# 10258392511/InverseProblemWithDiffusionModel

Hardware: AMD Instinct MI355X
Metric: ALD reconstructions/sec (128x128 complex, R=40, 4-coil) (higher is better)
Workload: dtype f32 (convolutions: operands as two fp16 pieces = 22 significand bits + 2 signs, three fp16 MFMAs per product, fp32 accumulate; every image scaled into fp16's range by an exact power of two from its producer's per-image maxima: any fp32 input, DESIGN.md 4.2); 1 GPU; ACDC-style 128x128 complex SENSE R=40 4-coil ALD reconstruction, NCSNv2Deepest ngf=128 (94.1M params, seeded random init), sigma 348->0.01 x 2311 levels x 3 steps, L2Penalty, denoise; 14 posterior samples = 14 on rank 0 + 13 per further rank (the 105-sample / 8-GPU partition of BASELINE config 3); samples_total=14, samples_this_rank=14, parallelism=sample-sharded x1, hip_graph=True, state_finite=True

## Files before the change

include/ipdm.h:

```cpp
#ifndef IPDM_H
#define IPDM_H

#include <stddef.h>
#include <stdint.h>

#ifdef __cplusplus
extern "C" {
#endif

#define IPDM_OK 0
#define IPDM_EINVAL (-1)
#define IPDM_EUNSUPPORTED (-2)

#define IPDM_ACT_NONE 0
#define IPDM_ACT_ELU 1
#define IPDM_ACT_RELU 2
#define IPDM_ACT_LRELU02 3
#define IPDM_ACT_SWISH 4
#define IPDM_ACT_COPY 5

#define IPDM_AMAX_WAYS 8
#define IPDM_AMAX_SLOT 128

#define IPDM_ABI_VERSION 4
// ... 215 lines not shown
                           int64_t n_samples, int64_t sample_elems, void* stream);

int ipdm_philox_normal_f32(float* out, uint64_t seed, int64_t sample_offset, int64_t step_id, int plane,
                           int64_t n_samples, int64_t sample_elems, void* stream);

int ipdm_philox_block_host(uint64_t seed, int64_t sample, int64_t step_id, int plane, uint32_t quad, uint32_t* out4);


int ipdm_instnorm_plus_coef_f32(const float* x, const float* alpha, const float* gamma, const float* beta,
                                float* coef, int B, int C, int HW,
                                float* amax_bound ,
                                void* stream);
int ipdm_cond_instnorm_plus_coef_f32(const float* x, const float* embed, const int64_t* labels, int num_classes, int bias,
                                     float* coef, int B, int C, int HW, float* amax_bound, void* stream);
int ipdm_affine_act_f32(const float* x, const float* coef, float* y, int B, int C, int HW, int act, void* stream);
int ipdm_act_f32(const float* x, float* y, int64_t n, int act, void* stream);
int ipdm_scale_shift_f32(const float* x, float* y, int64_t n, float a, float b, void* stream);
int ipdm_add_f32(const float* x, const float* y, float* out, int64_t n, void* stream);
int ipdm_div_sigma_f32(const float* x, const float* sigmas, const int64_t* labels, float* out,
                       int B, int64_t sample_elems, void* stream);
int ipdm_conv3x3_thin_supported(int Cin, int Cout, int H, int W);
int ipdm_conv3x3_thin_f32(const float* x, const float* w, const float* bias,
                          const float* coef ,
                          float* out, int B, int Cin, int Cout, int H, int W, void* stream);
int ipdm_conv3x3_thin_stats_partials(int Cin, int Cout, int H, int W);
int ipdm_conv3x3_thin_stats_f32(const float* x, const float* w, const float* bias, const float* coef, float* out, float* part,
                                int B, int Cin, int Cout, int H, int W, void* stream);
int ipdm_conv3x3_fewout_fin_supported(int Cin, int Cout, int H, int W);
int ipdm_conv3x3_fewout_fin_f32(const float* x, const float* w, const float* bias, const float* coef, int act, float* out,
                                int B, int Cin, int Cout, int H, int W, void* stream);
// ... 89 lines not shown
int ipdm_conv2d_wino_bx3_stats_partials(int Cin, int Cout, int H, int W, int dilation, int pool2);
int ipdm_conv2d_wino_bx3_stats_f32(const float* x, const void* U, const float* bias, const float* residual, float* out,
                                   float* out_act, int act_out, int B, int Cin, int Cout, int H, int W, int dilation,
                                   int pool2, float* stats, const ipdm_conv_ext_t* ext, void* stream);
int ipdm_absmax_f32(const float* x, float* amax , int n_images,
                    int64_t per_image, void* stream);
int64_t ipdm_conv_hx2_weight_bytes(int Cout, int Cin, int k);
int ipdm_conv_hx2_pack_weight(const float* w , void* packed, int Cout,
                              int Cin, int k, void* stream);
int ipdm_conv2d_hx2_f32(const float* x, const void* packed, const float* bias, const float* coef, int act,
                        const float* residual, float* out, float* out_act, int act_out,
                        int B, int Cin, int Cout, int H, int W, int k, int dilation, const ipdm_conv_ext_t* ext, void* stream);
int ipdm_conv3d_hx2_f32(const float* x, const void* packed, const float* bias, const float* coef, int act,
                        const float* residual, float* out, float* out_act, int act_out,
                        int B, int Cin, int Cout, int D, int H, int W, int k, int dilation, const ipdm_conv_ext_t* ext, void* stream);
int ipdm_conv_hx2_splitk_f32(const float* x, const void* packed, const float* bias, const float* coef, int act,
                             const float* residual, float* out, float* out_act, int act_out,
                             int B, int Cin, int Cout, int D, int H, int W, int k, int dilation, int volume, int ksplit,
                             float* work, const ipdm_conv_ext_t* ext, void* stream);
int64_t ipdm_conv_wino_hx2_weight_bytes(int Cout, int Cin);
int ipdm_conv_wino_hx2_pack_weight(const float* w , void* U, int Cout, int Cin, void* stream);
int ipdm_conv2d_wino_hx2_f32(const float* x, const void* U, const float* bias, const float* residual, float* out,
                             float* out_act, int act_out, int B, int Cin, int Cout, int H, int W, int dilation,
                             int pool2, const ipdm_conv_ext_t* ext, void* stream);
#define IPDM_WINO_FORM_OTHER 0
#define IPDM_WINO_FORM_CO32 1
#define IPDM_WINO_FORM_HALF 2
#define IPDM_WINO_FORM_POLY 3
int ipdm_conv2d_wino_hx2_form(int Cin, int Cout, int H, int W, int dilation);
int64_t ipdm_conv_wino1d_weight_bytes(int Cout, int Cin);
// ... 69 lines not shown
```

inverseproblemwithdiffusionmodel_amd/_lib.py:

```python
import ctypes
import os

import torch
from ctypes import c_char_p, c_double, c_float, c_int, c_int64, c_uint64, c_void_p


class ConvExt(ctypes.Structure):
    _fields_ = [("in_amax", c_void_p), ("bias_bstride", c_int), ("out_scale", c_float), ("res_second", c_int),
                ("out_amax", c_void_p), ("act_amax", c_void_p)]


_HERE = os.path.dirname(os.path.abspath(__file__))
LIB_PATH = os.environ.get("IPDM_LIB") or os.path.join(_HERE, "libipdm.so")

P = c_void_p

SIGNATURES = {
    "ipdm_abi_version": [],
    "ipdm_build_arch": [],
    "ipdm_upfirdn2d_f32": [P, P, P] + [c_int] * 14 + [P],
    "ipdm_fused_bias_act_f32": [P, P, P, P, c_int64, c_int, c_int, c_int, c_int, c_float, c_float, P],
    "ipdm_upfirdn2d_f16": [P, P, P] + [c_int] * 14 + [P],
    "ipdm_upfirdn2d_f64": [P, P, P] + [c_int] * 14 + [P],
    "ipdm_fused_bias_act_f16": [P, P, P, P, c_int64, c_int, c_int, c_int, c_int, c_float, c_float, P],
# ... 62 lines not shown
    "ipdm_pc_langevin_coef_f32": [P, P, P, P, c_double, c_double, c_uint64, c_int64, c_int64, P, c_float, c_float, P, P,
                                  c_int, c_int64, P],
    "ipdm_pc_sense_step_f32": [P, P, P, P, P, P, c_float, c_float, c_uint64, c_int64, c_int64, P, c_int,
                               P, P, c_int, c_int, P, c_int, c_float, P, c_int, c_int, c_int, c_int, P],
    "ipdm_pc_sense_cg_step_f32": [P, P, P, P, P, P, c_float, c_float, c_uint64, c_int64, c_int64, P, c_int,
                                  P, P, c_int, c_int, P, c_int, c_float, P, P, c_int, c_float, P,
                                  c_int, c_int, c_int, c_int, P],
    "ipdm_pc_singlecoil_step_f32": [P, P, P, P, P, P, c_float, c_float, c_uint64, c_int64, c_int64, P, c_int,
                                    P, P, c_int, c_float, c_int, P, c_int, c_int, c_int, P],
    "ipdm_langevin_step_f32": [P, P, P, c_float, c_float, c_uint64, c_int64, c_int64, P, c_int64, c_int64, P],
    "ipdm_philox_normal_f32": [P, c_uint64, c_int64, c_int64, c_int, c_int64, c_int64, P],
    "ipdm_philox_block_host": [c_uint64, c_int64, c_int64, c_int, ctypes.c_uint32, P],
    "ipdm_instnorm_plus_coef_f32": [P, P, P, P, P, c_int, c_int, c_int, P, P],
    "ipdm_cond_instnorm_plus_coef_f32": [P, P, P, c_int, c_int, P, c_int, c_int, c_int, P, P],
    "ipdm_affine_act_f32": [P, P, P, c_int, c_int, c_int, c_int, P],
    "ipdm_act_f32": [P, P, c_int64, c_int, P],
    "ipdm_scale_shift_f32": [P, P, c_int64, c_float, c_float, P],
    "ipdm_add_f32": [P, P, P, c_int64, P],
    "ipdm_div_sigma_f32": [P, P, P, P, c_int, c_int64, P],
    "ipdm_maxpool5_f32": [P, P, c_int, c_int, c_int, P],
    "ipdm_affine_avgpool5_f32": [P, P, P, c_int, c_int, c_int, P],
    "ipdm_meanpool2_f32": [P, P, c_int, c_int, c_int, P],
    "ipdm_bilinear_f32": [P, P, c_int, c_int, c_int, c_int, c_int, c_int, c_int, c_int, P, P],
    "ipdm_conv3x3_thin_supported": [c_int, c_int, c_int, c_int],
    "ipdm_conv3x3_thin_f32": [P, P, P, P, P, c_int, c_int, c_int, c_int, c_int, P],
    "ipdm_conv3x3_thin_stats_partials": [c_int, c_int, c_int, c_int],
    "ipdm_conv3x3_thin_stats_f32": [P, P, P, P, P, P, c_int, c_int, c_int, c_int, c_int, P],
    "ipdm_conv3x3_fewout_fin_supported": [c_int, c_int, c_int, c_int],
    "ipdm_conv3x3_fewout_fin_f32": [P, P, P, P, c_int, P, c_int, c_int, c_int, c_int, c_int, P],
    "ipdm_trilinear_f32": [P, P, c_int, c_int, c_int, c_int, c_int, c_int, c_int, c_int, c_int, c_int, P, P],
# ... 24 lines not shown
    "ipdm_conv_bx3_splitk_f32": [P, P, P, P, c_int, P, P, P, c_int] + [c_int] * 10 + [P, P, P],
    "ipdm_adam_ascent_f32": [P, P, P, P, c_int64, c_float, c_float, c_float, c_float, c_int, P],
    "ipdm_conv_wino_bx3_weight_bytes": [c_int, c_int],
    "ipdm_conv_wino_bx3_pack_weight": [P, P, c_int, c_int, P],
    "ipdm_conv2d_wino_bx3_supported": [c_int, c_int, c_int, c_int, c_int],
    "ipdm_conv2d_wino_bx3_f32": [P, P, P, P, P, P, c_int, c_int, c_int, c_int, c_int, c_int, c_int, c_int, P, P],
    "ipdm_conv2d_wino_bx3_stats_partials": [c_int, c_int, c_int, c_int, c_int, c_int],
    "ipdm_conv2d_wino_bx3_splitk": [c_int, c_int, c_int, c_int, c_int],
    "ipdm_conv2d_wino_bx3_splitk_f32": [P, P, P, P, P, P, c_int, c_int, c_int, c_int, c_int, c_int, c_int, c_int, P, P, P],
    "ipdm_conv2d_wino_bx3_stats_f32": [P, P, P, P, P, P, c_int, c_int, c_int, c_int, c_int, c_int, c_int, c_int, P, P, P],
    "ipdm_conv_hx2_weight_bytes": [c_int, c_int, c_int],
    "ipdm_conv_hx2_pack_weight": [P, P, c_int, c_int, c_int, P],
    "ipdm_absmax_f32": [P, P, c_int, c_int64, P],
    "ipdm_conv2d_hx2_f32": [P, P, P, P, c_int, P, P, P, c_int] + [c_int] * 7 + [P, P],
    "ipdm_conv3d_hx2_f32": [P, P, P, P, c_int, P, P, P, c_int] + [c_int] * 8 + [P, P],
    "ipdm_conv_hx2_splitk_f32": [P, P, P, P, c_int, P, P, P, c_int] + [c_int] * 10 + [P, P, P],
    "ipdm_conv_wino_hx2_weight_bytes": [c_int, c_int],
    "ipdm_conv_wino1d_weight_bytes": [c_int, c_int],
    "ipdm_conv_wino1d_pack_weight": [P, P, c_int, c_int, P],
    "ipdm_conv2d_wino1d_supported": [c_int, c_int, c_int, c_int],
    "ipdm_conv_wino1d_weight_bytes3d": [c_int, c_int],
    "ipdm_conv_wino1d_pack_weight3d": [P, P, c_int, c_int, P],
    "ipdm_conv3d_wino1d_supported": [c_int, c_int, c_int, c_int, c_int],
    "ipdm_conv3d_wino1d_f32": [P, P, P, P, P, P, c_int, c_int, c_int, c_int, c_int, c_int, c_int, P, P],
    "ipdm_conv2d_wino1d_f32": [P, P, P, P, c_int, P, P, P, c_int, c_int, c_int, c_int, c_int, c_int, c_int, P, P],
    "ipdm_conv2d_wino1d_stats_partials": [c_int, c_int, c_int, c_int],
    "ipdm_conv2d_wino1d_stats_f32": [P, P, P, P, c_int, P, P, P, c_int, c_int, c_int, c_int, c_int, c_int, c_int, P, P, P],
    "ipdm_conv_wino_hx2_pack_weight": [P, P, c_int, c_int, P],
    "ipdm_conv2d_wino_hx2_f32": [P, P, P, P, P, P, c_int, c_int, c_int, c_int, c_int, c_int, c_int, c_int, P, P],
    "ipdm_conv2d_wino_hx2_form": [c_int] * 5,
# ... 74 lines not shown
```

inverseproblemwithdiffusionmodel_amd/csrc/conv_bx3.hip:

```cpp
#include "conv_kernel.h"

namespace ipdm_conv {

constexpr int BX3_KG = 8;

template <int NCT, int NPT, int WCO, int WPX, int PW, int DMAX, int KS, bool HX = false, int ZT = 1>
struct BxCfg {
  static constexpr int NPC = HX ? 2 : 3;
  static constexpr int TAPS = KS * KS;
  static constexpr int CO_T = 32 * NCT * WCO;
  static constexpr int ROWS_PER_TILE = 32 / PW;
  static constexpr int PH = NPT * WPX * ROWS_PER_TILE;
  static constexpr int HALO = KS == 3 ? DMAX : 0;
  static constexpr int PHP = PH + 2 * HALO;
  static constexpr int PWP = PW + 2 * HALO;
  static constexpr int PITCH = PW == 32 ? PWP : (PWP + 15) / 16 * 16;
  static constexpr int PLANE_S = PHP * PITCH;
  static constexpr int PLANE = ZT * PLANE_S;
  static constexpr int STAGE = 2 * NPC * PLANE;
  static constexpr int ITEMS = (2 * ZT * PHP * PWP + 255) / 256;
  static constexpr int NPT_T = NPT * ZT;
  static constexpr size_t LDS_BYTES = 2 * (size_t)STAGE * 16;
};

// ... 718 lines not shown
```

inverseproblemwithdiffusionmodel_amd/csrc/conv_kernel.h:

```cpp
#pragma once
#include "launch.h"
#include <cstddef>
#include <cstdlib>
#include <type_traits>
#include <utility>

namespace ipdm_conv {

typedef float f32x16 __attribute__((ext_vector_type(16)));
typedef __bf16 bf16x8 __attribute__((ext_vector_type(8)));

__device__ __forceinline__ void split3(const float (&v)[8], bf16x8& h, bf16x8& m, bf16x8& l) {
#pragma unroll
  for (int i = 0; i < 8; ++i) {
    const __bf16 hi = (__bf16)v[i];
    const float r1 = v[i] - (float)hi;
    const __bf16 mi = (__bf16)r1;
    const float r2 = r1 - (float)mi;
    h[i] = hi;
    m[i] = mi;
    l[i] = (__bf16)r2;
  }
}

// ... 47 lines not shown
  (f(std::integral_constant<int, Is>{}), ...);
}
template <int N, typename F>
__device__ __forceinline__ void static_for(F&& f) {
  static_for_impl(f, std::make_integer_sequence<int, N>{});
}

__device__ __forceinline__ float half_wave_sum(float v) {
  v += __builtin_bit_cast(float, __builtin_amdgcn_update_dpp(0, __builtin_bit_cast(int, v), 0xB1, 0xf, 0xf, false));
  v += __builtin_bit_cast(float, __builtin_amdgcn_update_dpp(0, __builtin_bit_cast(int, v), 0x4E, 0xf, 0xf, false));
  v += __builtin_bit_cast(float, __builtin_amdgcn_update_dpp(0, __builtin_bit_cast(int, v), 0x141, 0xf, 0xf, false));
  v += __builtin_bit_cast(float, __builtin_amdgcn_update_dpp(0, __builtin_bit_cast(int, v), 0x140, 0xf, 0xf, false));
  return v + __shfl_xor(v, 16, 64);
}


struct ConvArgs {
  const float* x = nullptr;
  const float* wt = nullptr;
  const float* bias = nullptr;
  const float* coef = nullptr;
  const float* residual = nullptr;
  float* out = nullptr;
  float* out_act = nullptr;
  int act_out = IPDM_ACT_NONE;
  int B = 0, Cin = 0, Cout = 0, H = 0, W = 0, dil = 1, act = IPDM_ACT_NONE;
  int D = 1, kd = 1;
  int tiles_x = 0, tiles_y = 0, co_tiles = 0;
  unsigned long long* dbg = nullptr;
  int pool2 = 0;
// ... 392 lines not shown
```

inverseproblemwithdiffusionmodel_amd/csrc/norm_act.hip:

```cpp
#include "ipdm_common.h"

namespace {

template <bool REG>
__global__ __launch_bounds__(256) void plane_stats_kernel(const float* __restrict__ x, float* __restrict__ coef,
                                                          int HW) {
  __shared__ double red[4];
  const float* p = x + (size_t)blockIdx.x * HW;
  const int tid = threadIdx.x, lane = tid & 63, wave = tid >> 6;
  const bool vec = REG || ((HW % 4 == 0) && ((reinterpret_cast<uintptr_t>(p) & 15) == 0));
  float4 keep[16];
  float s = 0.f;
  if constexpr (REG) {
    const int n4 = HW / 4;
#pragma unroll
    for (int k = 0; k < 16; ++k) {
      const int i = tid + k * 256;
      keep[k] = i < n4 ? reinterpret_cast<const float4*>(p)[i] : make_float4(0.f, 0.f, 0.f, 0.f);
    }
#pragma unroll
    for (int k = 0; k < 16; ++k)
      if (tid + k * 256 < n4) s += (keep[k].x + keep[k].y) + (keep[k].z + keep[k].w);
  } else if (vec) {
    for (int i = tid; i < HW / 4; i += 256) {
// ... 174 lines not shown
  const size_t plane = blockIdx.y;
  const float mu = coef[plane * 3], sc = coef[plane * 3 + 1], sh = coef[plane * 3 + 2];
  const float* p = x + plane * HW;
  float* o = y + plane * HW;
  if ((HW & 3) == 0 && ((reinterpret_cast<uintptr_t>(p) | reinterpret_cast<uintptr_t>(o)) & 15) == 0) {
    for (int i = blockIdx.x * 256 + threadIdx.x; i < HW / 4; i += gridDim.x * 256) {
      float4 v = reinterpret_cast<const float4*>(p)[i];
      v.x = ipdm_act((v.x - mu) * sc + sh, act);
      v.y = ipdm_act((v.y - mu) * sc + sh, act);
      v.z = ipdm_act((v.z - mu) * sc + sh, act);
      v.w = ipdm_act((v.w - mu) * sc + sh, act);
      reinterpret_cast<float4*>(o)[i] = v;
    }
  } else {
    for (int i = blockIdx.x * 256 + threadIdx.x; i < HW; i += gridDim.x * 256) o[i] = ipdm_act((p[i] - mu) * sc + sh, act);
  }
}

__global__ __launch_bounds__(256) void affine_act_cat_kernel(const float* x1, int C1, const float* x2, int C2,
                                                             const float* __restrict__ coef, float* y, int HW, int act) {
  const size_t plane = blockIdx.y;
  const int Ct = C1 + C2;
  const size_t b = plane / Ct;
  const int c = (int)(plane % Ct);
  const float mu = coef[plane * 3], sc = coef[plane * 3 + 1], sh = coef[plane * 3 + 2];
  const float* p = c < C1 ? x1 + (b * C1 + c) * HW : x2 + (b * C2 + (c - C1)) * HW;
  float* o = y + plane * HW;
  if ((HW & 3) == 0 && ((reinterpret_cast<uintptr_t>(p) | reinterpret_cast<uintptr_t>(o)) & 15) == 0) {
    for (int i = blockIdx.x * 256 + threadIdx.x; i < HW / 4; i += gridDim.x * 256) {
      float4 v = reinterpret_cast<const float4*>(p)[i];
// ... 389 lines not shown
  if (B == 0) return IPDM_OK;
  IPDM_REQUIRE(x && coef && y);
  IPDM_REQUIRE((int64_t)B * C <= 65535 * 32);
  int gx = (HW / 4 + 255) / 256;
  if (gx < 1) gx = 1;
  if (gx > 64) gx = 64;
  int64_t planes = (int64_t)B * C;
  for (int64_t p0 = 0; p0 < planes; p0 += 65535) {
    int np = (int)((planes - p0) < 65535 ? (planes - p0) : 65535);
    hipLaunchKernelGGL(affine_act_kernel, dim3(gx, np), dim3(256), 0, ipdm_stream(stream), x + p0 * HW, coef + p0 * 3,
                       y + p0 * HW, HW, act);
  }
  return ipdm_launch_status();
}

extern "C" int ipdm_affine_act_cat_f32(const float* x1, int C1, const float* x2, int C2, const float* coef, float* y, int B,
                                       int HW, int act, void* stream) {
  IPDM_REQUIRE(B >= 0 && C1 > 0 && C2 > 0 && HW > 0);
  if (B == 0) return IPDM_OK;
  IPDM_REQUIRE(x1 && x2 && coef && y && y != x1 && y != x2);
  const int64_t planes = (int64_t)B * (C1 + C2);
  if (planes > 65535) return IPDM_EUNSUPPORTED;
  int gx = (HW / 4 + 255) / 256;
  gx = gx < 1 ? 1 : (gx > 64 ? 64 : gx);
  hipLaunchKernelGGL(affine_act_cat_kernel, dim3(gx, (unsigned)planes), dim3(256), 0, ipdm_stream(stream), x1, C1, x2, C2, coef,
                     y, HW, act);
  return ipdm_launch_status();
}

extern "C" int ipdm_act_f32(const float* x, float* y, int64_t n, int act, void* stream) {
// ... 174 lines not shown
```

inverseproblemwithdiffusionmodel_amd/ncsn/models/layers.py:

```python
import os
from functools import partial

import torch
import torch.nn as nn

from ... import ops, _lib
from .normalization import InstanceNorm2dPlus, ConditionalInstanceNorm2dPlus, get_normalization


class _Act:

    def __init__(self, name):
        self.name = name
        self.code = ops.ACT_CODES[name]

    def __call__(self, x):
        return ops.act(x, self.code)


USE_WINOGRAD = os.environ.get("IPDM_WINOGRAD", "1") != "0"
FUSE_POOL = os.environ.get("IPDM_FUSE_POOL", "1") != "0"


def get_act(config):
# ... 131 lines not shown
def _maxpool(x):
    if x.dim() == 3:
        return ops.maxpool1d5(x)
    return ops.maxpool3d5(x) if x.dim() == 5 else ops.maxpool5(x)


class ConvMeanPool(nn.Module):
    def __init__(self, input_dim, output_dim, kernel_size=3, biases=True, adjust_padding=False, spec_norm=False, ndim=2):
        super().__init__()
        if adjust_padding or spec_norm:
            raise NotImplementedError("adjust_padding / spec_norm are unused by every shipped config")
        if ndim == 3:
            raise NotImplementedError("the 8-way 3-D ConvMeanPool is unused by NCSN3DShallow (all its stages are dilated)")
        self.conv = Conv2d(input_dim, output_dim, kernel_size, bias=biases, ndim=ndim)

    def forward(self, inputs, feeds_conv=True):
        if self.conv.ndim == 1:
            if self.conv.kernel_size == 1:
                return self.conv(ops.meanpool1d2(inputs), feeds_conv=feeds_conv)
            return ops.meanpool1d2(self.conv(inputs, feeds_conv=feeds_conv))
        if self.conv.kernel_size == 1:
            return self.conv(ops.meanpool2(inputs), feeds_conv=feeds_conv)
        return ops.meanpool2(self.conv(inputs, feeds_conv=feeds_conv))

    def fused(self, inputs, residual=None, act_out=ops.ACT_NONE, feeds_conv=True, coef=None, act=ops.ACT_NONE):
        c = self.conv
        route = c.route(inputs, site="pool", coef=coef, act=act, act_out=act_out)
        bias, dyn = None if c.bias is None else c.bias.data, ops.dynamic_range()
        if route is None:
            return None
        if route == ops.ROUTE_SEQ:
            return ops.conv1d(inputs, c.packed_conv1d(), bias, residual, c.dilation,
                              act_out=act_out, in_amax=ops.in_amax_for(inputs) if dyn else None, want_amax=dyn and feeds_conv,
                              pool2=True)
        try:
            if coef is not None:
                return ops.conv2d_wino_bx3(inputs, c.packed_wino1d(), bias, residual,
# ... 156 lines not shown
                self.normalize2 = normalization(output_dim)
                self.conv2 = dilated_conv3x3_(output_dim, output_dim, dilation=dilation, spec_norm=spec_norm)
            else:
                conv_shortcut = partial(conv1x1_, spec_norm=spec_norm)
                self.conv1 = conv3x3_(input_dim, output_dim, spec_norm=spec_norm)
                self.normalize2 = normalization(output_dim)
                self.conv2 = conv3x3_(output_dim, output_dim, spec_norm=spec_norm)
        else:
            raise Exception('invalid resample value')
        if output_dim != input_dim or resample is not None:
            self.shortcut = conv_shortcut(input_dim, output_dim)
        self.normalize1 = normalization(input_dim)

    def forward(self, x, want_act=False):
        code = _act_code(self.non_linearity)
        h = self._norm_act_conv(self.normalize1, self.conv1, x, code, want_stats=True, feeds_conv=False)
        a2 = None
        if self.output_dim == self.input_dim and self.resample is None:
            shortcut = x
        else:
            shortcut = self.shortcut(x, feeds_conv=False)
        if isinstance(self.conv2, ConvMeanPool):
            plain_norm = isinstance(self.normalize2, InstanceNorm2dPlus) and self.conv2.conv.ndim == 2
            coef2 = self.normalize2.coef(h) if plain_norm else None
            fin = plain_norm and code == ops.ACT_ELU and self.conv2.conv.fuses_input(h, coef2)
            a2 = h if fin else (ops.affine_act(h, coef2, code) if plain_norm else self.normalize2(h, code))
            fused = self.conv2.fused(a2, residual=shortcut, act_out=code if want_act else ops.ACT_NONE, feeds_conv=want_act,
                                     coef=coef2 if fin else None, act=code if fin else ops.ACT_NONE)
            if fused is not None:
                return fused
            if fin:
                a2 = ops.affine_act(h, coef2, code)
            out = ops.add(shortcut, self.conv2(a2))
            return (out, ops.act(out, code)) if want_act else out
        if want_act:
            return self._norm_act_conv(self.normalize2, self.conv2, h, code, residual=shortcut, act_out=code, want_stats=True)
        return self._norm_act_conv(self.normalize2, self.conv2, h, code, residual=shortcut, want_stats=True, feeds_conv=False)

    @staticmethod
    def _norm_act_conv(norm, conv, x, code, **kw):
        if code == ops.ACT_ELU and isinstance(conv, Conv2d) and conv.ndim == 2 and isinstance(norm, InstanceNorm2dPlus):
            coef = norm.coef(x)
            if conv.fuses_input(x, coef):
                return conv(x, coef=coef, act=code, **kw)
            return conv(ops.affine_act(x, coef, code), **kw)
        return conv(norm(x, code), **kw)



def _cond_norm_act_conv(coef, conv, x, code, **kw):
    if code == ops.ACT_ELU and isinstance(conv, Conv2d) and conv.fuses_input(x, coef):
        return conv(x, coef=coef, act=code, **kw)
    return conv(ops.affine_act(x, coef, code), **kw)


class ConditionalResidualBlock(nn.Module):
    def __init__(self, input_dim, output_dim, num_classes, resample=None, act=None,
                 normalization=ConditionalInstanceNorm2dPlus, adjust_padding=False, dilation=None, spec_norm=False):
        super().__init__()
        self.non_linearity = act
        self.input_dim = input_dim
# ... 166 lines not shown
```

inverseproblemwithdiffusionmodel_amd/ops.py:

```python
import ctypes
import os

import torch

from . import _lib
from ._lib import call, P

ACT_NONE, ACT_ELU, ACT_RELU, ACT_LRELU02, ACT_SWISH = 0, 1, 2, 3, 4
ACT_COPY = 5
CONV_TRACE = None

ACT_CODES = {"none": ACT_NONE, None: ACT_NONE, "elu": ACT_ELU, "relu": ACT_RELU, "lrelu": ACT_LRELU02,
             "swish": ACT_SWISH}


def _gpu(t, dtype=None, name="tensor"):
    if not isinstance(t, torch.Tensor) or not t.is_cuda:
        raise RuntimeError(f"ipdm: {name} must be a GPU tensor (the HIP path has no CPU fallback); got "
                           f"{getattr(t, 'device', type(t))}")
    if dtype is not None and t.dtype != dtype:
        raise TypeError(f"ipdm: {name} must be {dtype}, got {t.dtype}")
    return t if t.is_contiguous() else t.contiguous()


# ... 1240 lines not shown
    part = getattr(x, "_ipdm_partials", None)
    if part is not None:
        del x._ipdm_partials
        part, tag = part
        if tag != (x._version, x.data_ptr()):
            part = None
    if part is not None and USE_STATS_EPILOGUE and tuple(part.shape[:2]) == (B, C):
        call("ipdm_cond_instnorm_plus_coef_partials_f32", _ptr(part), int(part.shape[2]), _ptr(embed), _ptr(labels), nc,
             int(bool(bias)), _ptr(coef), B, C, hw, _ptr(bound), _stream())
        return coef
    call("ipdm_cond_instnorm_plus_coef_f32", _ptr(x), _ptr(embed), _ptr(labels), nc, int(bool(bias)), _ptr(coef), B, C, hw,
         _ptr(bound), _stream())
    return coef


def affine_act(x, coef, act=ACT_NONE, out=None):
    x = _gpu(x, torch.float32, "x")
    B, C = x.shape[:2]
    out = torch.empty_like(x) if out is None else out
    call("ipdm_affine_act_f32", _ptr(x), _ptr(coef), _ptr(out), B, C, x.numel() // max(B * C, 1), act, _stream())
    _written(out)
    return tag_amax(out, getattr(coef, "_ipdm_amax_bound", None))


def act(x, code, out=None):
    x = _gpu(x, torch.float32, "x")
    out = torch.empty_like(x) if out is None else out
    call("ipdm_act_f32", _ptr(x), _ptr(out), x.numel(), code, _stream())
    am = amax_of(x)
    _written(out)
    return tag_amax(out, am)


def scale_shift(x, a, b, out=None):
    x = _gpu(x, torch.float32, "x")
    out = torch.empty_like(x) if out is None else out
    call("ipdm_scale_shift_f32", _ptr(x), _ptr(out), x.numel(), float(a), float(b), _stream())
# ... 554 lines not shown
        D = 1
    ksplit = _lib.lib.ipdm_conv_bx3_splitk(B, D, Cin, wq.Cout, H, W, k, dilation) if B else 1
    if ksplit > 1:
        work = torch.empty((ksplit,) + shape, dtype=torch.float32, device=x.device)
        call(f"ipdm_conv_{wq.fmt}_splitk_f32", _ptr(x), _ptr(wq.blob), _ptr(bias), _ptr(coef), act, _ptr(residual), _ptr(out),
             _ptr(out_act), act_out, B, Cin, wq.Cout, D, H, W, k, dilation, int(vol), ksplit, _ptr(work), ext, _stream())
    elif vol:
        call(f"ipdm_conv3d_{wq.fmt}_f32", _ptr(x), _ptr(wq.blob), _ptr(bias), _ptr(coef), act, _ptr(residual), _ptr(out),
             _ptr(out_act), act_out, B, Cin, wq.Cout, D, H, W, k, dilation, ext, _stream())
    else:
        call(f"ipdm_conv2d_{wq.fmt}_f32", _ptr(x), _ptr(wq.blob), _ptr(bias), _ptr(coef), act, _ptr(residual), _ptr(out),
             _ptr(out_act), act_out, B, Cin, wq.Cout, H, W, k, dilation, ext, _stream())
    _written(out)
    return _conv_done(e0, out, out_act, slot_o, slot_a, B=B * D, Cin=Cin, Cout=wq.Cout, H=H, W=W, k=k, dil=dilation, bx3=True,
                      fmt=wq.fmt, res=residual is not None, taps3d=wq.kk if vol else None)


def conv_wino_bx3_weight(w, fmt="bx3"):
    if fmt not in SPLIT_IMPLS:
        raise ValueError(f"conv_wino_bx3_weight: fmt {fmt!r}")
    w = _gpu(w, torch.float32, "weight")
    Cout, Cin = w.shape[:2]
    nbytes = getattr(_lib.lib, f"ipdm_conv_wino_{fmt}_weight_bytes")(Cout, Cin)
    blob = torch.empty(nbytes, dtype=torch.uint8, device=w.device)
    call(f"ipdm_conv_wino_{fmt}_pack_weight", _ptr(w), _ptr(blob), Cout, Cin, _stream())
    return PackedBx3(blob, Cout, Cin, 16, fmt)


def conv_wino_hx2_weight(w):
    return conv_wino_bx3_weight(w, fmt="hx2")
# ... 331 lines not shown
```

Measured before the change: 0.1257 reconstructions/s.

## Fuse shortcut meanpool into norm-act pass and add streaming 1x1 conv kernel

On downsampling residual blocks, the norm+ELU affine pass now also emits the 2x2 mean-pooled raw input, so the separate meanpool over the block input is dropped. The pooled tensor then goes to a new streaming 1x1 fp16x2 MFMA conv kernel that stages input channels through LDS, instead of the generic conv path. Both are on by default behind environment flags. The aim is to cut one full read of the activation and launch overhead on the shortcut branch, at the cost of a new kernel with its own tiling and precision path.

New measurement: 0.1268 reconstructions/s (median of 6 runs). No clear change (+0.8%).

```diff
diff --git a/include/ipdm.h b/include/ipdm.h
--- a/include/ipdm.h
+++ b/include/ipdm.h
@@ -253,6 +253,8 @@
 int ipdm_cond_instnorm_plus_coef_f32(const float* x, const float* embed, const int64_t* labels, int num_classes, int bias,
                                      float* coef, int B, int C, int HW, float* amax_bound, void* stream);
 int ipdm_affine_act_f32(const float* x, const float* coef, float* y, int B, int C, int HW, int act, void* stream);
+int ipdm_affine_act_pool2_f32(const float* x, const float* coef, float* y, float* pooled, int B, int C, int H, int W, int act,
+                              void* stream);
 int ipdm_act_f32(const float* x, float* y, int64_t n, int act, void* stream);
 int ipdm_scale_shift_f32(const float* x, float* y, int64_t n, float a, float b, void* stream);
 int ipdm_add_f32(const float* x, const float* y, float* out, int64_t n, void* stream);
@@ -372,6 +374,8 @@
 int ipdm_conv3d_hx2_f32(const float* x, const void* packed, const float* bias, const float* coef, int act,
                         const float* residual, float* out, float* out_act, int act_out,
                         int B, int Cin, int Cout, int D, int H, int W, int k, int dilation, const ipdm_conv_ext_t* ext, void* stream);
+int ipdm_conv1x1_stream_hx2_f32(const float* x, const void* packed, const float* bias, float* out, int B, int Cin, int Cout,
+                                int H, int W, const ipdm_conv_ext_t* ext, void* stream);
 int ipdm_conv_hx2_splitk_f32(const float* x, const void* packed, const float* bias, const float* coef, int act,
                              const float* residual, float* out, float* out_act, int act_out,
                              int B, int Cin, int Cout, int D, int H, int W, int k, int dilation, int volume, int ksplit,
diff --git a/inverseproblemwithdiffusionmodel_amd/_lib.py b/inverseproblemwithdiffusionmodel_amd/_lib.py
--- a/inverseproblemwithdiffusionmodel_amd/_lib.py
+++ b/inverseproblemwithdiffusionmodel_amd/_lib.py
@@ -100,6 +100,7 @@
     "ipdm_instnorm_plus_coef_f32": [P, P, P, P, P, c_int, c_int, c_int, P, P],
     "ipdm_cond_instnorm_plus_coef_f32": [P, P, P, c_int, c_int, P, c_int, c_int, c_int, P, P],
     "ipdm_affine_act_f32": [P, P, P, c_int, c_int, c_int, c_int, P],
+    "ipdm_affine_act_pool2_f32": [P, P, P, P, c_int, c_int, c_int, c_int, c_int, P],
     "ipdm_act_f32": [P, P, c_int64, c_int, P],
     "ipdm_scale_shift_f32": [P, P, c_int64, c_float, c_float, P],
     "ipdm_add_f32": [P, P, P, c_int64, P],
@@ -154,6 +155,7 @@
     "ipdm_absmax_f32": [P, P, c_int, c_int64, P],
     "ipdm_conv2d_hx2_f32": [P, P, P, P, c_int, P, P, P, c_int] + [c_int] * 7 + [P, P],
     "ipdm_conv3d_hx2_f32": [P, P, P, P, c_int, P, P, P, c_int] + [c_int] * 8 + [P, P],
+    "ipdm_conv1x1_stream_hx2_f32": [P, P, P, P, c_int, c_int, c_int, c_int, c_int, P, P],
     "ipdm_conv_hx2_splitk_f32": [P, P, P, P, c_int, P, P, P, c_int] + [c_int] * 10 + [P, P, P],
     "ipdm_conv_wino_hx2_weight_bytes": [c_int, c_int],
     "ipdm_conv_wino1d_weight_bytes": [c_int, c_int],
diff --git a/inverseproblemwithdiffusionmodel_amd/csrc/conv1x1_stream.hip b/inverseproblemwithdiffusionmodel_amd/csrc/conv1x1_stream.hip
--- /dev/null
+++ b/inverseproblemwithdiffusionmodel_amd/csrc/conv1x1_stream.hip
@@ -0,0 +1,212 @@
+#include "conv_kernel.h"
+
+namespace ipdm_conv {
+
+struct Conv1x1Args {
+  const float* x;
+  const uint4* wq;
+  const float* bias;
+  const float* in_amax;
+  float* out;
+  float out_scale;
+  int B, Cin, Cout, HW;
+  int n_pt, n_cg;
+};
+
+constexpr int S1_KB = 8;
+constexpr int S1_CT = 8;
+static_assert(S1_KB == BX3_KG, "an accumulation group of the grouped form ends where a staged block ends");
+
+template <int NPT>
+constexpr size_t s1_lds_bytes() { return (size_t)S1_KB * 2 * 2 * 32 * NPT * 16; }
+
+template <int NPT, bool GROUPED, bool DYN>
+__global__ __launch_bounds__(256, 2) void conv1x1_stream_kernel(Conv1x1Args a) {
+  constexpr int PT = 32 * NPT;
+  constexpr int ITEMS = S1_KB * 2 * PT / 256;
+  constexpr int CSTEP = 256 / (2 * PT);
+  static_assert(NPT == 2 || NPT == 4, "64 or 128 pixels per workgroup");
+  extern __shared__ __align__(16) uint4 lds4[];
+  const int tid = threadIdx.x, lane = tid & 63;
+  const int wave = __builtin_amdgcn_readfirstlane(tid >> 6);
+  const int h = lane >> 5, j = lane & 31;
+  const int HW = a.HW;
+  const int n_cc = a.Cin / 16, n_ct = a.Cout / 32;
+  int u = blockIdx.x;
+  const int cg = u % a.n_cg;
+  u /= a.n_cg;
+  const int pt = u % a.n_pt;
+  const int b = u / a.n_pt;
+
+  float hx_in = 1.f, hx_out = 1.f;
+  if constexpr (DYN) hx_dynamic_scale(ipdm_amax_read_v(a.in_amax + (size_t)b * IPDM_AMAX_SLOT), hx_in, hx_out);
+
+  const int sp = tid % PT, sg = (tid / PT) & 1, sc0 = tid / (2 * PT);
+  const int spix = pt * PT + sp;
+  const int sofs = 8 * sg * HW + (spix < HW ? spix : HW - 1);
+  const float* const xb = a.x + (size_t)b * a.Cin * HW;
+  float xr[ITEMS][8];
+  auto load_block = [&](int c0) {
+#pragma unroll
+    for (int k = 0; k < ITEMS; ++k) {
+      const int c = c0 + sc0 + k * CSTEP, cc = c < n_cc ? c : n_cc - 1;
+#pragma unroll
+      for (int q = 0; q < 8; ++q) xr[k][q] = (xb + (size_t)(cc * 16 + q) * HW)[sofs];
+    }
+  };
+  auto store_block = [&]() {
+#pragma unroll
+    for (int k = 0; k < ITEMS; ++k) {
+      uint4 ph, pl;
+      if constexpr (DYN) split2_scaled(xr[k], hx_in, ph, pl);
+      else split2(xr[k], ph, pl);
+      const int at = ((sc0 + k * CSTEP) * 4 + sg) * PT + sp;
+      lds4[at] = ph;
+      lds4[at + 2 * PT] = pl;
+    }
+  };
+
+  int ct_ofs[2];
+#pragma unroll
+  for (int m = 0; m < 2; ++m) {
+    const int ct = cg * S1_CT + 2 * wave + m;
+    ct_ofs[m] = (ct < n_ct ? ct : n_ct - 1) * 128 + lane;
+  }
+  auto load_A = [&](uint4 (&fr)[2][2], int cc) {
+    const uint4* p = a.wq + (size_t)(cc < n_cc ? cc : n_cc - 1) * n_ct * 128;
+#pragma unroll
+    for (int m = 0; m < 2; ++m) {
+      fr[m][0] = p[ct_ofs[m]];
+      fr[m][1] = p[ct_ofs[m] + 64];
+    }
+  };
+
+  f32x16 acc[2][NPT];
+  f32x16 tot[GROUPED ? 2 : 1][GROUPED ? NPT : 1];
+#pragma unroll
+  for (int m = 0; m < 2; ++m)
+#pragma unroll
+    for (int n = 0; n < NPT; ++n)
+#pragma unroll
+      for (int r = 0; r < 16; ++r) {
+        acc[m][n][r] = 0.f;
+        if constexpr (GROUPED) tot[m][n][r] = 0.f;
+      }
+
+  uint4 afr[2][2][2];
+  const int b_rd = h * PT + j;
+  auto chunk = [&](auto pc, int cl, int cc) {
+    constexpr int p = decltype(pc)::value;
+    load_A(afr[p ^ 1], cc + 1);
+    __builtin_amdgcn_sched_barrier(0);
+    const uint4* bp = lds4 + cl * 4 * PT + b_rd;
+#pragma unroll
+    for (int n = 0; n < NPT; ++n) {
+      const f16x8 bh = __builtin_bit_cast(f16x8, bp[n * 32]), bl = __builtin_bit_cast(f16x8, bp[2 * PT + n * 32]);
+#pragma unroll
+      for (int m = 0; m < 2; ++m) {
+        const f16x8 ah = __builtin_bit_cast(f16x8, afr[p][m][0]), al = __builtin_bit_cast(f16x8, afr[p][m][1]);
+        f32x16 c = acc[m][n];
+        c = __builtin_amdgcn_mfma_f32_32x32x16_f16(al, bh, c, 0, 0, 0);
+        c = __builtin_amdgcn_mfma_f32_32x32x16_f16(ah, bl, c, 0, 0, 0);
+        c = __builtin_amdgcn_mfma_f32_32x32x16_f16(ah, bh, c, 0, 0, 0);
+        acc[m][n] = c;
+      }
+    }
+    __builtin_amdgcn_sched_barrier(0);
+  };
+
+  load_A(afr[0], 0);
+  for (int c0 = 0; c0 < n_cc; c0 += S1_KB) {
+    load_block(c0);
+    if (c0) __syncthreads();
+    store_block();
+    __syncthreads();
+    const int kb = n_cc - c0 < S1_KB ? n_cc - c0 : S1_KB;
+    int cl = 0;
+    for (; cl + 1 < kb; cl += 2) {
+      chunk(std::integral_constant<int, 0>{}, cl, c0 + cl);
+      chunk(std::integral_constant<int, 1>{}, cl + 1, c0 + cl + 1);
+    }
+    if (cl < kb) chunk(std::integral_constant<int, 0>{}, cl, c0 + cl);
+    if constexpr (GROUPED) {
+#pragma unroll
+      for (int m = 0; m < 2; ++m)
+#pragma unroll
+        for (int n = 0; n < NPT; ++n)
+#pragma unroll
+          for (int r = 0; r < 16; ++r) {
+            tot[m][n][r] += acc[m][n][r];
+            acc[m][n][r] = 0.f;
+          }
+    }
+  }
+
+  const float* const scale_p = reinterpret_cast<const float*>(a.wq + (size_t)n_cc * n_ct * 128);
+  const bool has_bias = a.bias != nullptr;
+  const float* const bias_p = has_bias ? a.bias : scale_p;
+  float* const ob = a.out + (size_t)b * a.Cout * HW;
+#pragma unroll
+  for (int m = 0; m < 2; ++m) {
+    const int ct = cg * S1_CT + 2 * wave + m;
+    if (ct >= n_ct) break;
+    float sv[16], bv[16];
+#pragma unroll
+    for (int r = 0; r < 16; ++r) {
+      const int co = ct * 32 + (r & 3) + 8 * (r >> 2) + 4 * h;
+      sv[r] = scale_p[co] * hx_out;
+      bv[r] = bias_p[co];
+    }
+#pragma unroll
+    for (int n = 0; n < NPT; ++n) {
+      const int pix = pt * PT + n * 32 + j;
+      if (pix >= HW) continue;
+      const int oofs = 4 * h * HW + pix;
+#pragma unroll
+      for (int r = 0; r < 16; ++r) {
+        float* const oc = ob + (size_t)(ct * 32 + (r & 3) + 8 * (r >> 2)) * HW;
+        float v;
+        if constexpr (GROUPED) v = tot[m][n][r];
+        else v = acc[m][n][r];
+        v *= sv[r];
+        const float vb = v + bv[r];
+        v = has_bias ? vb : v;
+        v *= a.out_scale;
+        oc[oofs] = v;
+      }
+    }
+  }
+}
+
+template <int NPT, bool GROUPED>
+static int launch_conv1x1_stream(Conv1x1Args a, hipStream_t s) {
+  a.n_pt = (a.HW + 32 * NPT - 1) / (32 * NPT);
+  a.n_cg = (a.Cout / 32 + S1_CT - 1) / S1_CT;
+  const int64_t nblk = (int64_t)a.B * a.n_pt * a.n_cg;
+  if (nblk > 0x7fffffff) return IPDM_EUNSUPPORTED;
+  if (a.in_amax)
+    return ipdm_launch_lds(conv1x1_stream_kernel<NPT, GROUPED, true>, dim3((unsigned)nblk), dim3(256), s1_lds_bytes<NPT>(), s, a);
+  return ipdm_launch_lds(conv1x1_stream_kernel<NPT, GROUPED, false>, dim3((unsigned)nblk), dim3(256), s1_lds_bytes<NPT>(), s, a);
+}
+
+}
+
+using namespace ipdm_conv;
+
+extern "C" int ipdm_conv1x1_stream_hx2_f32(const float* x, const void* packed, const float* bias, float* out, int B, int Cin,
+                                           int Cout, int H, int W, const ipdm_conv_ext_t* ext, void* stream) {
+  IPDM_REQUIRE(B >= 0 && Cin > 0 && Cout > 0 && H > 0 && W > 0);
+  if (B == 0) return IPDM_OK;
+  IPDM_REQUIRE(x && packed && out && x != out);
+  if (Cin % 16 || Cout % 32 || ((reinterpret_cast<uintptr_t>(x) | reinterpret_cast<uintptr_t>(out)) & 15)) return IPDM_EUNSUPPORTED;
+  if (ext && (ext->bias_bstride || ext->res_second || ext->out_amax || ext->act_amax)) return IPDM_EUNSUPPORTED;
+  if ((int64_t)H * W >= (1 << 26)) return IPDM_EUNSUPPORTED;
+  Conv1x1Args a;
+  a.x = x; a.wq = static_cast<const uint4*>(packed); a.bias = bias; a.out = out;
+  a.in_amax = ext ? ext->in_amax : nullptr;
+  a.out_scale = ext && ext->out_scale != 0.f ? ext->out_scale : 1.f;
+  a.B = B; a.Cin = Cin; a.Cout = Cout; a.HW = H * W;
+  a.n_pt = a.n_cg = 0;
+  const bool grouped = W <= 16 && Cin / 16 > BX3_KG;
+  return grouped ? launch_conv1x1_stream<2, true>(a, ipdm_stream(stream)) : launch_conv1x1_stream<4, false>(a, ipdm_stream(stream));
+}
diff --git a/inverseproblemwithdiffusionmodel_amd/csrc/conv_bx3.hip b/inverseproblemwithdiffusionmodel_amd/csrc/conv_bx3.hip
--- a/inverseproblemwithdiffusionmodel_amd/csrc/conv_bx3.hip
+++ b/inverseproblemwithdiffusionmodel_amd/csrc/conv_bx3.hip
@@ -1,8 +1,6 @@
 #include "conv_kernel.h"
 
 namespace ipdm_conv {
-
-constexpr int BX3_KG = 8;
 
 template <int NCT, int NPT, int WCO, int WPX, int PW, int DMAX, int KS, bool HX = false, int ZT = 1>
 struct BxCfg {
diff --git a/inverseproblemwithdiffusionmodel_amd/csrc/conv_kernel.h b/inverseproblemwithdiffusionmodel_amd/csrc/conv_kernel.h
--- a/inverseproblemwithdiffusionmodel_amd/csrc/conv_kernel.h
+++ b/inverseproblemwithdiffusionmodel_amd/csrc/conv_kernel.h
@@ -85,6 +85,8 @@
   return v + __shfl_xor(v, 16, 64);
 }
 
+
+constexpr int BX3_KG = 8;
 
 struct ConvArgs {
   const float* x = nullptr;
diff --git a/inverseproblemwithdiffusionmodel_amd/csrc/norm_act.hip b/inverseproblemwithdiffusionmodel_amd/csrc/norm_act.hip
--- a/inverseproblemwithdiffusionmodel_amd/csrc/norm_act.hip
+++ b/inverseproblemwithdiffusionmodel_amd/csrc/norm_act.hip
@@ -212,6 +212,38 @@
     }
   } else {
     for (int i = blockIdx.x * 256 + threadIdx.x; i < HW; i += gridDim.x * 256) o[i] = ipdm_act((p[i] - mu) * sc + sh, act);
+  }
+}
+
+__global__ __launch_bounds__(256) void affine_act_pool2_kernel(const float* __restrict__ x, const float* __restrict__ coef,
+                                                               float* __restrict__ y, float* __restrict__ pooled, int H, int W,
+                                                               int act) {
+  const size_t plane = blockIdx.y;
+  const float mu = coef[plane * 3], sc = coef[plane * 3 + 1], sh = coef[plane * 3 + 2];
+  const int HW = H * W, qw = W / 4, items = (H / 2) * qw;
+  const float* p = x + plane * HW;
+  float* o = y + plane * HW;
+  float* po = pooled + plane * (HW / 4);
+  for (int i = blockIdx.x * 256 + threadIdx.x; i < items; i += gridDim.x * 256) {
+    const int r = i / qw, q = i - r * qw;
+    const int at = 2 * r * W + 4 * q;
+    const float4 top = *reinterpret_cast<const float4*>(p + at);
+    const float4 bot = *reinterpret_cast<const float4*>(p + at + W);
+    float4 v;
+    v.x = ipdm_act((top.x - mu) * sc + sh, act);
+    v.y = ipdm_act((top.y - mu) * sc + sh, act);
+    v.z = ipdm_act((top.z - mu) * sc + sh, act);
+    v.w = ipdm_act((top.w - mu) * sc + sh, act);
+    *reinterpret_cast<float4*>(o + at) = v;
+    v.x = ipdm_act((bot.x - mu) * sc + sh, act);
+    v.y = ipdm_act((bot.y - mu) * sc + sh, act);
+    v.z = ipdm_act((bot.z - mu) * sc + sh, act);
+    v.w = ipdm_act((bot.w - mu) * sc + sh, act);
+    *reinterpret_cast<float4*>(o + at + W) = v;
+    float2 m;
+    m.x = (((top.x + bot.x) + top.y) + bot.y) / 4.0f;
+    m.y = (((top.z + bot.z) + top.w) + bot.w) / 4.0f;
+    *reinterpret_cast<float2*>(po + r * (W / 2) + 2 * q) = m;
   }
 }
 
@@ -631,6 +663,26 @@
   return ipdm_launch_status();
 }
 
+extern "C" int ipdm_affine_act_pool2_f32(const float* x, const float* coef, float* y, float* pooled, int B, int C, int H, int W,
+                                         int act, void* stream) {
+  IPDM_REQUIRE(B >= 0 && C > 0 && H > 0 && W > 0);
+  if (B == 0) return IPDM_OK;
+  IPDM_REQUIRE(x && coef && y && pooled && x != y && x != pooled && y != pooled);
+  IPDM_REQUIRE((int64_t)B * C <= 65535 * 32 && (int64_t)H * W <= 0x7fffffff);
+  if (H % 2 || W % 4 || ((reinterpret_cast<uintptr_t>(x) | reinterpret_cast<uintptr_t>(y) | reinterpret_cast<uintptr_t>(pooled)) & 15))
+    return IPDM_EUNSUPPORTED;
+  const int HW = H * W, items = HW / 8;
+  int gx = (items + 255) / 256;
+  gx = gx < 1 ? 1 : (gx > 64 ? 64 : gx);
+  const int64_t planes = (int64_t)B * C;
+  for (int64_t p0 = 0; p0 < planes; p0 += 65535) {
+    const int np = (int)((planes - p0) < 65535 ? (planes - p0) : 65535);
+    hipLaunchKernelGGL(affine_act_pool2_kernel, dim3(gx, np), dim3(256), 0, ipdm_stream(stream), x + p0 * HW, coef + p0 * 3,
+                       y + p0 * HW, pooled + p0 * (HW / 4), H, W, act);
+  }
+  return ipdm_launch_status();
+}
+
 extern "C" int ipdm_affine_act_cat_f32(const float* x1, int C1, const float* x2, int C2, const float* coef, float* y, int B,
                                        int HW, int act, void* stream) {
   IPDM_REQUIRE(B >= 0 && C1 > 0 && C2 > 0 && HW > 0);
diff --git a/inverseproblemwithdiffusionmodel_amd/ncsn/models/layers.py b/inverseproblemwithdiffusionmodel_amd/ncsn/models/layers.py
--- a/inverseproblemwithdiffusionmodel_amd/ncsn/models/layers.py
+++ b/inverseproblemwithdiffusionmodel_amd/ncsn/models/layers.py
@@ -169,13 +169,18 @@
             raise NotImplementedError("the 8-way 3-D ConvMeanPool is unused by NCSN3DShallow (all its stages are dilated)")
         self.conv = Conv2d(input_dim, output_dim, kernel_size, bias=biases, ndim=ndim)
 
-    def forward(self, inputs, feeds_conv=True):
+    def forward(self, inputs, feeds_conv=True, pooled=None, stream=False):
         if self.conv.ndim == 1:
             if self.conv.kernel_size == 1:
                 return self.conv(ops.meanpool1d2(inputs), feeds_conv=feeds_conv)
             return ops.meanpool1d2(self.conv(inputs, feeds_conv=feeds_conv))
         if self.conv.kernel_size == 1:
-            return self.conv(ops.meanpool2(inputs), feeds_conv=feeds_conv)
+            c = self.conv
+            pooled = ops.meanpool2(inputs) if pooled is None else pooled
+            if stream and not feeds_conv and ops.CONV_IMPL == "hx2" and not c.full_range and ops.conv1x1_stream_ok(c.packed(), pooled):
+                return ops.conv1x1_stream(pooled, c.packed(), None if c.bias is None else c.bias.data,
+                                          in_amax=ops.in_amax_for(pooled) if ops.dynamic_range() else None)
+            return c(pooled, feeds_conv=feeds_conv)
         return ops.meanpool2(self.conv(inputs, feeds_conv=feeds_conv))
 
     def fused(self, inputs, residual=None, act_out=ops.ACT_NONE, feeds_conv=True, coef=None, act=ops.ACT_NONE):
@@ -362,10 +367,18 @@
 
     def forward(self, x, want_act=False):
         code = _act_code(self.non_linearity)
-        h = self._norm_act_conv(self.normalize1, self.conv1, x, code, want_stats=True, feeds_conv=False)
+        sc = getattr(self, "shortcut", None)
+        down = isinstance(sc, ConvMeanPool) and sc.conv.kernel_size == 1 and sc.conv.ndim == 2
+        pooled = None
+        if down and ops.SHORTCUT_POOL:
+            h, pooled = self._norm_act_conv(self.normalize1, self.conv1, x, code, pool2=True, want_stats=True, feeds_conv=False)
+        else:
+            h = self._norm_act_conv(self.normalize1, self.conv1, x, code, want_stats=True, feeds_conv=False)
         a2 = None
         if self.output_dim == self.input_dim and self.resample is None:
             shortcut = x
+        elif down:
+            shortcut = sc(x, feeds_conv=False, pooled=pooled, stream=True)
         else:
             shortcut = self.shortcut(x, feeds_conv=False)
         if isinstance(self.conv2, ConvMeanPool):
@@ -386,13 +399,20 @@
         return self._norm_act_conv(self.normalize2, self.conv2, h, code, residual=shortcut, want_stats=True, feeds_conv=False)
 
     @staticmethod
-    def _norm_act_conv(norm, conv, x, code, **kw):
+    def _norm_act_conv(norm, conv, x, code, pool2=False, **kw):
+        pooled = None
         if code == ops.ACT_ELU and isinstance(conv, Conv2d) and conv.ndim == 2 and isinstance(norm, InstanceNorm2dPlus):
             coef = norm.coef(x)
             if conv.fuses_input(x, coef):
-                return conv(x, coef=coef, act=code, **kw)
-            return conv(ops.affine_act(x, coef, code), **kw)
-        return conv(norm(x, code), **kw)
+                out = conv(x, coef=coef, act=code, **kw)
+            elif pool2:
+                a, pooled = ops.affine_act(x, coef, code, pool2=True)
+                out = conv(a, **kw)
+            else:
+                out = conv(ops.affine_act(x, coef, code), **kw)
+        else:
+            out = conv(norm(x, code), **kw)
+        return (out, pooled) if pool2 else out
 
 
 
diff --git a/inverseproblemwithdiffusionmodel_amd/ops.py b/inverseproblemwithdiffusionmodel_amd/ops.py
--- a/inverseproblemwithdiffusionmodel_amd/ops.py
+++ b/inverseproblemwithdiffusionmodel_amd/ops.py
@@ -1278,13 +1278,26 @@
     return coef
 
 
-def affine_act(x, coef, act=ACT_NONE, out=None):
+SHORTCUT_POOL = os.environ.get("IPDM_SHORTCUT_POOL", "1") != "0"
+
+
+def affine_act(x, coef, act=ACT_NONE, out=None, pool2=False):
     x = _gpu(x, torch.float32, "x")
     B, C = x.shape[:2]
     out = torch.empty_like(x) if out is None else out
+    bound = getattr(coef, "_ipdm_amax_bound", None)
+    if pool2:
+        H, W = x.shape[2:]
+        if H % 2 == 0 and W % 4 == 0 and out.data_ptr() != x.data_ptr() and (x.data_ptr() | out.data_ptr()) % 16 == 0:
+            pooled = torch.empty((B, C, H // 2, W // 2), dtype=torch.float32, device=x.device)
+            call("ipdm_affine_act_pool2_f32", _ptr(x), _ptr(coef), _ptr(out), _ptr(pooled), B, C, H, W, act, _stream())
+            _written(out)
+            return tag_amax(out, bound), carry_amax(x, pooled)
+        pooled = meanpool2(x)
     call("ipdm_affine_act_f32", _ptr(x), _ptr(coef), _ptr(out), B, C, x.numel() // max(B * C, 1), act, _stream())
     _written(out)
-    return tag_amax(out, getattr(coef, "_ipdm_amax_bound", None))
+    out = tag_amax(out, bound)
+    return (out, pooled) if pool2 else out
 
 
 def act(x, code, out=None):
@@ -1869,6 +1882,31 @@
     _written(out)
     return _conv_done(e0, out, out_act, slot_o, slot_a, B=B * D, Cin=Cin, Cout=wq.Cout, H=H, W=W, k=k, dil=dilation, bx3=True,
                       fmt=wq.fmt, res=residual is not None, taps3d=wq.kk if vol else None)
+
+
+CONV1X1_STREAM = os.environ.get("IPDM_CONV1X1_STREAM", "1") != "0"
+
+
+def conv1x1_stream_ok(wq, x):
+    return (CONV1X1_STREAM and isinstance(wq, PackedBx3) and wq.fmt == "hx2" and wq.kk == 1 and x.dim() == 4
+            and wq.Cin % 16 == 0 and wq.Cout % 32 == 0 and x.data_ptr() % 16 == 0)
+
+
+def conv1x1_stream(x, wq, bias=None, in_amax=None, out_scale=1.0):
+    x = _gpu(x, torch.float32, "x")
+    if not isinstance(wq, PackedBx3) or wq.fmt != "hx2" or wq.kk != 1 or x.dim() != 4:
+        raise _lib.IpdmUnsupported("conv1x1_stream: an f16x2 1x1 blob and a [B,Cin,H,W] input")
+    if bias is not None and bias.dim() != 1:
+        raise _lib.IpdmUnsupported("conv1x1_stream: per-channel bias only")
+    if wq.Cin != x.shape[1]:
+        raise ValueError(f"conv1x1_stream: weight Cin {wq.Cin} != input Cin {x.shape[1]}")
+    B, Cin, H, W = x.shape
+    out = torch.empty((B, wq.Cout, H, W), dtype=torch.float32, device=x.device)
+    ext = _conv_ext("hx2", in_amax, x, False, out_scale=out_scale)
+    e0 = _trace_open()
+    call("ipdm_conv1x1_stream_hx2_f32", _ptr(x), _ptr(wq.blob), _ptr(bias), _ptr(out), B, Cin, wq.Cout, H, W, ext, _stream())
+    return _conv_done(e0, out, None, B=B, Cin=Cin, Cout=wq.Cout, H=H, W=W, k=1, dil=1, bx3=True, fmt="hx2", res=False,
+                      taps3d=None, stream=True)
 
 
 def conv_wino_bx3_weight(w, fmt="bx3"):
```
